# michalfratczak/habdec

Measured on AMD Instinct MI355X. Metric: IQ Msamples/s (batched 2.048 MS/s streams), higher is better.
Workload: dtype f32

## Files before the change

### habdec_amd/csrc/engine.cpp

```cpp
#include <hip/hip_runtime.h>
#include <rocfft/rocfft.h>

#include <algorithm>
#include <atomic>
#include <chrono>
#include <cmath>
#include <cstdio>
#include <cstdlib>
#include <cstring>
#include <memory>
#include <condition_variable>
#include <mutex>
#include <thread>
#include <string>
#include <vector>

#include "../../include/habdec_amd.h"
#include "dev_types.h"
#include "host/afc_tracker.hpp"
#include "host/decim_plan.hpp"
#include "host/fir_design.hpp"
#include "host/iq_file_batch.hpp"
#include "host/text_stage.hpp"
#include "host/tune_host.hpp"
#include "kernels/launch.h"

#define HDK(fn, ...) (e->fast ? hd::fast::fn(__VA_ARGS__) : hd::exact::fn(__VA_ARGS__))

namespace {

thread_local std::string g_err;
int fail(int code, const std::string& msg) { g_err = msg; return code; }

#define HD_HIP(call)                                                                                   \
    do {                                                                                               \
        hipError_t e_ = (call);                                                                        \
        if (e_ != hipSuccess) return fail(HD_ERR_DEVICE, std::string(#call) + ": " + hipGetErrorString(e_)); \
    } while (0)

template <typename T>
// ... 83 lines not shown
    int bins_sep = 8;
    bool decode_enabled = true;
    bool fast = false;
    bool one_stream = false;
    bool no_tail = false;
    uint32_t tail_max_n2 = 2048;
    int last_route = -1;
    struct PendingTail { bool valid = false; hd::TailArgs ta{}; int slot = 0; bool any_fft = false; int r2 = 0, t2 = 0; } pend;
    bool own_fft = false;
    bool tail_fft = true;
    DevBuf<float2> fft_tw;
    bool no_claim = false;
    uint32_t step_run = 0;
    bool no_cu_step = false;
    uint32_t ring_run = 0;
    uint32_t ring_short_pct = 25;
    static constexpr uint32_t kS1Loaders = 2;
#ifndef HD_S1_SLOTS_BATCH
#define HD_S1_SLOTS_BATCH 4
#endif
    static constexpr uint32_t kS1Slots = HD_S1_SLOTS_BATCH;
    PinBuf<unsigned int> ring_gave_up;
    std::string fail_cause;
    bool device_failed = false;
    uint64_t step_launches = 0;
    DevBuf<unsigned int> step_ctr;
    uint32_t pend_max_taps = 0;
    bool dec_wgs_forced = false;
#ifdef HD_TIMING_EXPERIMENT
    int cu_exp = 0;
// ... 160 lines not shown
        const float rel = (float)(500.0f / e->fsd);
        e->bins_sep = std::max(8, (int)std::round((double)rel * (double)hd::kFftBins));
    }

    int ndev = 0;
    if (hipGetDeviceCount(&ndev) != hipSuccess || ndev <= cfg->device || cfg->device < 0)
        return fail(HD_ERR_DEVICE, "no HIP device " + std::to_string(cfg->device) + " (this library has no CPU path)");
    HD_HIP(hipSetDevice(cfg->device));
    HD_HIP(hipStreamCreateWithFlags(&e->qa, hipStreamNonBlocking));
    e->one_stream = cfg->pipeline == 0;
    e->no_tail = getenv("HD_NO_TAIL") != nullptr;
    e->no_claim = getenv("HD_NO_CLAIM") != nullptr;
    if (const char* v = getenv("HD_STEP_RUN")) e->step_run = (uint32_t)atoi(v);
    e->no_cu_step = getenv("HD_NO_CU_STEP") != nullptr;
    if (const char* v = getenv("HD_RING_RUN")) e->ring_run = (uint32_t)atoi(v);
    if (const char* v = getenv("HD_RING_SHORT_PCT")) e->ring_short_pct = std::min<uint32_t>((uint32_t)atoi(v), 100u);
    if (const char* v = getenv("HD_TAIL_MAX_N2")) e->tail_max_n2 = (uint32_t)strtoul(v, nullptr, 0);
    {
        hipDeviceProp_t prop;
        HD_HIP(hipGetDeviceProperties(&prop, cfg->device));
        e->n_cus = (uint32_t)prop.multiProcessorCount;
        e->dec_wgs_per_cu = cfg->pipeline ? 6u : 8u;
        if (const char* v = getenv("HD_DEC_WGS_PER_CU")) { e->dec_wgs_per_cu = (uint32_t)atoi(v); e->dec_wgs_forced = true; }
#ifdef HD_TIMING_EXPERIMENT
        if (const char* v = getenv("HD_CU_EXP")) e->cu_exp = atoi(v);
#endif
    }
    for (hipEvent_t* ev : {&e->ev_copy[0], &e->ev_copy[1], &e->ev_staging_free[0], &e->ev_staging_free[1]}) HD_HIP(hipEventCreateWithFlags(ev, hipEventDisableTiming));
    if (e->one_stream) e->qb = e->qc = e->qa;
    else {
// ... 627 lines not shown
{
    t.dec1 = b.d1; t.dec1_stride = e->n1_cap; t.hist2_in = e->hist2[b.hin].p; t.hist2_out = e->hist2[b.hout].p; t.taps2 = e->stage_taps[1].p;
    t.fbuf = b.fcur; t.fbuf_next = b.fnext; t.fbuf_stride = e->fbuf_stride; t.fir_hist_cap = e->fir_hist_cap;
    t.lp_taps = e->lp_taps.p; t.taps_stride = e->taps_cap; t.demod = e->demod.p; t.demod_stride = e->demod.n / e->S;
    t.filtered = e->cfg.keep_filtered ? e->filtered.p : nullptr; t.carry_in = e->carry[b.cin].p; t.carry_out = e->carry[b.cout].p;
    t.tune = p.any_tune ? sl.h_tune.dev : nullptr; t.tune_tab = e->tune_tab.p;
    t.call = r.dcall; t.fft_in = r.feed; t.head_buf = e->fir_head.p; t.fbuf_prev = b.fprev; t.head_cap = e->head_cap;
    t.n_streams = e->S;
    t.ring = e->tail.p; t.ring_cap = e->tail_cap; t.sym = e->d_symstate.p; t.flipmask = e->flipmask.p; t.wsum = e->weight.p;
    t.sp = e->d_sym.p; t.slots = sl.h_slots.dev; t.slot_words = e->slot_words; t.seq = sl.seq;
    t.flips_dbg = e->flips_cap ? e->flips_dbg.p : nullptr; t.flips_cap = e->flips_cap;
    const bool in_tail = e->tail_fft && e->cfg.enable_spectrum && r.feed;
    t.fft_tw = in_tail ? e->fft_tw.p : nullptr; t.spec = e->spec.p; t.power = e->power.p; t.stats = sl.h_stats.dev; t.rate = e->fsd; t.bins_sep = e->bins_sep;
}

hd::StepClaim make_claim(const hd_engine* e, const CallPlan& p, uint32_t lin_wgs ,
                         uint32_t run_len_cu )
{
    hd::StepClaim claim{};
    const int R1 = (int)p.R1, T1 = (int)p.T1;
    const uint64_t S = e->S;
    const uint32_t ntiles = run_len_cu ? HDK(ring_tiles, R1, T1, p.max_in) : (p.max_n1 + 63) / 64, n_xcd = e->n_cus / 32u, run_len = run_len_cu ? run_len_cu : e->step_run >= 2 ? e->step_run : 4u;
    const uint64_t runs = S * ntiles / run_len;
    const bool shape_ok = run_len_cu ? (HDK(stage1_cu_supported, R1, T1) && p.max_in % 2048u == 0) : ((R1 == 32 || R1 == 64) && p.max_n1 % 64 == 0);
    if (!e->no_claim && (p.nst == 2 || (run_len_cu && p.nst == 1)) && shape_ok && p.min_in == p.max_in && p.max_in && !p.any_zero1 && n_xcd && e->n_cus % 32u == 0 && n_xcd <= 16 &&
        ntiles && (ntiles % run_len == 0 || (run_len_cu && R1 >= 32 && (S * ntiles) % run_len == 0)) && runs % n_xcd == 0 && S * ntiles < (1ull << 32) && (uint64_t)ntiles * S >= 4ull * lin_wgs) {
        claim.ctr = e->step_ctr.p + (size_t)(e->step_launches & 1u) * 16 * 32;
        claim.ctr_next = e->step_ctr.p + (size_t)((e->step_launches & 1u) ^ 1u) * 16 * 32;
        claim.n_xcd = n_xcd; claim.runs_per_xcd = (uint32_t)(runs / n_xcd); claim.run_len = run_len;
        if (run_len_cu && R1 >= 32 && e->ring_short_pct) {
            const uint32_t tpx = claim.runs_per_xcd * run_len, whole = (uint32_t)((uint64_t)tpx * (100u - e->ring_short_pct) / 100u) / run_len;
            claim.tiles_per_xcd = tpx; claim.short_from = whole; claim.runs_per_xcd = whole + (tpx - whole * run_len);
        }
    }
    return claim;
}

uint32_t pick_ring_run(const hd_engine* e, uint32_t R1, uint32_t ntiles)
{
    const uint64_t S = e->S;
    const uint32_t n_xcd = e->n_cus / 32u ? e->n_cus / 32u : 1u, want = R1 >= 32 ? 4u : 8u;
    auto ok = [&](uint32_t r) { return r >= 2u && r <= ntiles && (R1 >= 32 ? (S * ntiles) % r == 0 : ntiles % r == 0) && (S * ntiles / r) % n_xcd == 0; };
    if (e->ring_run >= 2 && ok(e->ring_run)) return e->ring_run;
    for (uint32_t d = 0; d <= 8u; ++d) {
        if (ok(want + d)) return want + d;
        if (d && d < want && ok(want - d)) return want - d;
    }
// ... 57 lines not shown
        hd::TailArgs tacu{};
        if (HDK(tail_layout, tacu, 64, R2, T2, p.max_taps, e->max_R, e->min_R, e->tail_cap, p.max_pend, cu_tail)) r.ta_step = tacu;
    }
    fill_tail(e, sl, p, r, b, r.ta_step);
    hd_engine::PendingTail prev = e->pend;
    hd_engine::CallSlot* ps = prev.valid ? &e->slot[prev.slot] : nullptr;
    bool ev_on_dispatch = false;
    const int cu_exp = e->cu_exp;
    const bool want_cu = cu_tail && ((cu_exp & 1) || (r.ta_step.lds_bytes <= cu_tail && (!prev.valid || prev.ta.lds_bytes <= cu_tail)));
    const hd::StepClaim claim = make_claim(e, p, 0, want_cu ? ring_run : 0u);
    bool launched = false;
    e->last_timing.step_variant = 0;
    if (want_cu && claim.ctr) {
        const uint32_t tb = std::max(r.ta_step.lds_bytes, prev.valid ? prev.ta.lds_bytes : 0u);
        hd::StepClaim cl = claim;
        if (cu_exp & 2) { cl.runs_per_xcd = 0; cl.tiles_per_xcd = 0; cl.short_from = 0xFFFFFFFFu; }
        ev_on_dispatch = !ps || prev.ta.fft_tw || !prev.any_fft;
        if (sl.timed && !ev_on_dispatch) HD_HIP(hipEventRecord(sl.t1, qa));
        launched = HDK(launch_step_cu, qa, R1, T1, prev.valid ? prev.r2 : R2, prev.valid ? prev.t2 : T2, S, e->n_cus, iq, stride,
                                      e->hist1[b.hin].p, e->hist1[b.hout].p, e->stage_taps[0].p, b.d1, e->n1_cap, sl.h_call.dev, sl.d_call.p, prev.ta,
                                      (prev.valid && !(cu_exp & 1)) ? S : 0u, p.max_in, cl, tb,
                                      ev_on_dispatch && sl.timed ? sl.t1 : nullptr, !ev_on_dispatch ? nullptr : sl.timed ? sl.t2 : ps ? ps->ev_done : nullptr);
        if (!launched && ev_on_dispatch) { ev_on_dispatch = false; if (sl.timed) HD_HIP(hipEventRecord(sl.t1, qa)); }
        e->last_timing.step_variant = launched ? 1u : 0u;
    }
    else if (sl.timed) HD_HIP(hipEventRecord(sl.t1, qa));
    if (launched) ++e->step_launches;
    else {
        const hd::StepClaim fb = (want_cu && claim.ctr) ? hd::StepClaim{} : claim;
        const uint32_t wgs = (fb.ctr ? 8u : 32u) * e->n_cus;
        if (prev.valid && prev.ta.lds_bytes > HDK(step_lds_bytes, R1, T1)) {
// ... 509 lines not shown
```

### habdec_amd/csrc/kernels/decimate.hip

```cpp
#include <hip/hip_runtime.h>
#include <hip/hip_ext.h>
#include <type_traits>
#include <cstdlib>

#include "launch.h"
#include "tune.h"
#include "tail_body.h"
#include "stage1_ring.h"

#define HD_DEC_MAXW 4

namespace hd {
namespace HD_ARITH_NS {

#ifdef HD_STAMP_DEC
#ifndef HD_STAMP_DEC_D
#define HD_STAMP_DEC_D 32
#endif
__device__ unsigned long long g_dec_stamps[4096 * 8];
extern "C" void HD_DBG_NAME(hd_debug_dec_stamps)(unsigned long long* host, size_t n) { (void)hipMemcpyFromSymbol(host, HIP_SYMBOL(g_dec_stamps), n * 8); }
#define DSTAMP_DECL unsigned long long ds_t = __builtin_amdgcn_s_memtime(), ds_acc[4] = {0, 0, 0, 0}; const unsigned long long ds_r0 = __builtin_amdgcn_s_memrealtime(); unsigned long long ds_r1 = 0
#define DSTAMP(i) do { if (D == HD_STAMP_DEC_D) { const unsigned long long t_ = __builtin_amdgcn_s_memtime(); ds_acc[i] += t_ - ds_t; ds_t = t_; } } while (0)
#define DSTAMP_ARRIVED() do { if (D == HD_STAMP_DEC_D) { asm volatile("s_waitcnt vmcnt(0)" ::: "memory"); DSTAMP(0); if (!ds_r1) ds_r1 = __builtin_amdgcn_s_memrealtime(); } } while (0)
#define DSTAMP_WRITE() do { if (D == HD_STAMP_DEC_D && threadIdx.x == 0) { const uint32_t w_ = by * gdx + bx; if (w_ < 4096) { \
// ... 620 lines not shown
                           out_stride, call, n_streams, ntiles, call_copy, ta, n_tail, uniform_n, claim);                             \
        return true;                                                                                                                  \
    }
    HD_STEP_CASE(32, 212, 2, 69) HD_STEP_CASE(32, 174, 4, 139) HD_STEP_CASE(64, 348, 4, 139)
#undef HD_STEP_CASE
    return false;
}

uint32_t ring_tiles(int ratio, int ntaps, uint32_t n)
{
    if (ratio != 32 && ratio != 64) return n / 2048u;
    const uint32_t adv = 64u - (uint32_t)((ntaps - 1 + ratio - 1) / ratio), rows = n / (uint32_t)ratio;
    return rows >= 64u ? (rows + adv - 1u) / adv : 0u;
}

static bool ring_limits_ok(uint32_t ntiles, const StepClaim& claim, bool workers = false )
{
    const uint64_t total = claim.tiles_per_xcd ? (uint64_t)claim.tiles_per_xcd * claim.n_xcd : (uint64_t)claim.runs_per_xcd * claim.n_xcd * claim.run_len;
    if (workers) return ntiles && claim.run_len >= 2u && total % ntiles == 0 && total < (1ull << 32) &&
                        (!claim.tiles_per_xcd || (uint64_t)claim.tiles_per_xcd == (uint64_t)(claim.short_from < claim.runs_per_xcd ? claim.short_from : claim.runs_per_xcd) * claim.run_len +
                                                                                    (claim.runs_per_xcd - (claim.short_from < claim.runs_per_xcd ? claim.short_from : claim.runs_per_xcd)));
    return ntiles && ntiles <= 4096u && claim.run_len && ntiles % claim.run_len == 0 && total < (1ull << 24) && total / ntiles <= (1ull << 20);
}

uint32_t step_cu_tail_lds(int ratio, int ntaps)
{
    if (ratio != 32 || (ntaps != 212 && ntaps != 174)) return 0;
    return ((163840u - (uint32_t)kRingCtlBytes - 4u * (uint32_t)kWorkSlotBytes) / 4u) & ~15u;
}

bool launch_step_cu(hipStream_t st, int ratio, int ntaps, int ratio2, int ntaps2, uint32_t n_streams, uint32_t n_cus, const float2* in, size_t in_stride,
                    const float2* hist_in, float2* hist_out, const float* taps, float2* out, size_t out_stride, const StreamCall* call,
                    StreamCall* call_copy, const TailArgs& ta, uint32_t n_tail, uint32_t uniform_n, const StepClaim& claim, uint32_t tail_bytes,
                    hipEvent_t ev_start, hipEvent_t ev_stop)
{
    if (ratio != 32 || !claim.ctr || !uniform_n || uniform_n % 2048u) return false;
    const uint32_t ntiles = ring_tiles(ratio, ntaps, uniform_n);
    if (!ring_limits_ok(ntiles, claim, true)) return false;
    if (tail_bytes < (uint32_t)kWorkSlotBytes) tail_bytes = (uint32_t)kWorkSlotBytes;
    tail_bytes = (tail_bytes + 15u) & ~15u;
    RingArgs ra{in, in_stride, hist_in, hist_out, taps, out, out_stride, uniform_n, ntiles, claim, nullptr, nullptr, 0u, nullptr};
#define HD_CU_CASE(T, D2, T2)                                                                                                         \
    if (ntaps == T && ratio2 == D2 && ntaps2 == T2) {                                                                                 \
        const uint32_t lds = (uint32_t)kRingCtlBytes + (n_tail ? 4u * (uint32_t)kWorkSlotBytes + 4u * tail_bytes : 8u * (uint32_t)kWorkSlotBytes); \
        if (lds > 163840u) return false;                                                                                              \
        static bool attr_set[64] = {};                              \
        int dev_ = 0;                                                                                                                 \
        if (hipGetDevice(&dev_) != hipSuccess || dev_ < 0 || dev_ >= 64) return false;                                                \
        if (!attr_set[dev_]) {                                                                                                        \
            if (hipFuncSetAttribute(reinterpret_cast<const void*>(k_step_cu<T, D2, T2>), hipFuncAttributeMaxDynamicSharedMemorySize, 163840) != hipSuccess) return false; \
            attr_set[dev_] = true;                                                                                                    \
        }                                                                                                                             \
        const dim3 grid_(n_cus > (n_streams + 3u) / 4u ? n_cus : (n_streams + 3u) / 4u);                                             \
// ... 18 lines not shown
}

bool launch_stage1_cu(hipStream_t st, int ratio, int ntaps, uint32_t n_cus, const float2* in, size_t in_stride, const float2* hist_in, float2* hist_out,
                      const float* taps, float2* out, size_t out_stride, uint32_t uniform_n, const StepClaim& claim, unsigned int* gave_up, uint32_t n_loaders, uint32_t n_waves,
                      uint32_t n_slots, const StreamCall* final_call, uint32_t fir_hist_cap, float2* fft_in)
{
    if (n_loaders != 1u) n_loaders = 2u;
    if (ratio <= 4) {
        n_loaders = 1u;
        n_waves = 16u;
    }
    if (n_slots < 2u * n_loaders || n_slots > 8u) n_slots = 8u;
    if (n_waves < 8u || n_waves > 16u) n_waves = 8u;
    if (!claim.ctr || !uniform_n || uniform_n % 2048u) return false;
    const uint32_t ntiles = ring_tiles(ratio, ntaps, uniform_n);
    if (!ring_limits_ok(ntiles, claim, ratio >= 32)) return false;
    if ((ratio <= 4) != (final_call != nullptr)) return false;
    RingArgs ra{in, in_stride, hist_in, hist_out, taps, out, out_stride, uniform_n, ntiles, claim, gave_up, final_call, fir_hist_cap, fft_in};
#define HD_S1_CASE(D, T)                                                                                                              \
    if (ratio == D && ntaps == T) {                                                                                                   \
        static_assert(D >= 32 || (uint32_t)ring_bytes<T, kRingNSLAlone>() <= 163840u, "eight tile slots must fit a CU's LDS");       \
        const uint32_t workers = D == 32 ? 8u : n_slots <= 4u ? 3u : 4u;             \
        const uint32_t lds = D >= 32 ? workers * (uint32_t)work_slot_bytes<(D >= 32 ? D : 32)>() : n_slots * (uint32_t)ring_slot_bytes<T>() + (uint32_t)kRingCtlBytes; \
        static bool attr_set[64] = {};                                                                                                \
        int dev_ = 0;                                                                                                                 \
        if (hipGetDevice(&dev_) != hipSuccess || dev_ < 0 || dev_ >= 64) return false;                                                \
        if (!attr_set[dev_]) {                                                                                                        \
            if (hipFuncSetAttribute(reinterpret_cast<const void*>(k_stage1_cu<T, D>), hipFuncAttributeMaxDynamicSharedMemorySize, 163840) != hipSuccess) return false; \
            attr_set[dev_] = true;                                                                                                    \
        }                                                                                                                             \
        hipLaunchKernelGGL((k_stage1_cu<T, D>), dim3(n_cus), dim3(64u * (D == 4 ? n_waves : D >= 32 ? workers : 8u)), lds, st, ra, n_loaders, n_slots);   \
// ... 33 lines not shown
```

### habdec_amd/csrc/kernels/launch.h

```cpp
#pragma once
#include <hip/hip_runtime.h>
#include <stddef.h>
#include <stdint.h>

#include "../dev_types.h"

namespace hd {

struct DemodCarry {
    float re, im;
    uint32_t primed;
    uint32_t _pad;
};

struct StepClaim {
    unsigned int* ctr = nullptr;
    unsigned int* ctr_next = nullptr;
    uint32_t n_xcd = 0, runs_per_xcd = 0, run_len = 0;
    uint32_t short_from = 0xFFFFFFFFu, tiles_per_xcd = 0;
};

struct TailArgs {
    const float2* dec1; size_t dec1_stride;
    const float2* hist2_in; float2* hist2_out; const float* taps2;
    float2* fbuf; float2* fbuf_next; size_t fbuf_stride; uint32_t fir_hist_cap;
    const float* lp_taps; uint32_t taps_stride;
    float* demod; size_t demod_stride; float2* filtered;
    const DemodCarry* carry_in; DemodCarry* carry_out;
    const StreamCall* call; float2* fft_in;
    float2* head_buf ; const float2* fbuf_prev ; uint32_t head_cap, n_streams;
    float* ring; uint32_t ring_cap; SymState* sym; unsigned long long* flipmask; float* wsum; const SymbolParams* sp;
    uint32_t* slots; uint32_t slot_words; uint32_t* flips_dbg; uint32_t flips_cap;
    uint32_t seq;
    const float2* fft_tw; float2* spec; float* power; SpectrumStatsDev* stats; double rate; int bins_sep;
// ... 24 lines not shown
```

### habdec_amd/csrc/kernels/stage1_ring.h

```cpp
#pragma once
#include <hip/hip_runtime.h>

#include "arith.h"
#include "launch.h"

namespace hd {
namespace HD_ARITH_NS {

typedef float r_f32x2 __attribute__((ext_vector_type(2)));
typedef float r_f32x4 __attribute__((ext_vector_type(4)));

constexpr int kRingRowBytes = 272;
constexpr int kRingNSLAlone = 4;
constexpr int kWorkSlotBytes = 64 * kRingRowBytes;
constexpr int kRingCtlBytes = 384;
constexpr uint32_t kRingSpinLimit = 1u << 22;
template <int T> constexpr int ring_halo_rows() { return (T - 1 + 31) / 32; }
template <int T> constexpr int ring_slot_bytes() { return (64 + ring_halo_rows<T>()) * kRingRowBytes; }
template <int T, int NSL = kRingNSLAlone> constexpr int ring_bytes() { return 2 * NSL * ring_slot_bytes<T>() + kRingCtlBytes; }
template <int T> constexpr int ring_adv() { return 64 - ring_halo_rows<T>(); }

__host__ __device__ constexpr uint32_t ring_sys_tiles(uint32_t n, uint32_t adv) { return (n / 32u + adv - 1u) / adv; }

#ifdef HD_STAMP_RING
// ... 73 lines not shown
}

__device__ __forceinline__ void glds16(const void* base, uint32_t off, uint32_t lds_dst)
{
    unsigned keep;
    asm volatile("s_mov_b32 %0, m0\n\ts_mov_b32 m0, %3\n\ts_nop 0\n\tglobal_load_lds_dwordx4 %1, %2\n\ts_mov_b32 m0, %0"
                 : "=&s"(keep) : "v"(off), "s"(base), "s"(lds_dst) : "memory");
}
__device__ __forceinline__ void glds4(const void* base, uint32_t off, uint32_t lds_dst)
{
    unsigned keep;
    asm volatile("s_mov_b32 %0, m0\n\ts_mov_b32 m0, %3\n\ts_nop 0\n\tglobal_load_lds_dword %1, %2\n\ts_mov_b32 m0, %0"
                 : "=&s"(keep) : "v"(off), "s"(base), "s"(lds_dst) : "memory");
}

template <bool HEAD_KEPT = false >
__device__ __forceinline__ void glds16_x17(const void* base, const uint32_t (&off)[17], uint32_t lds_dst)
{
    unsigned keep, scc_keep;
#define HD_GLDS_BODY_POLICY " nt"
#define HD_G1(n) "global_load_lds_dwordx4 %" #n ", %19" HD_GLDS_BODY_POLICY "\n\ts_add_u32 m0, m0, 0x400\n\ts_nop 0\n\t"
#define HD_G1D(n) "global_load_lds_dwordx4 %" #n ", %19\n\ts_add_u32 m0, m0, 0x400\n\ts_nop 0\n\t"
#define HD_G17_OPS : "=&s"(keep), "=&s"(scc_keep)                                                                                                                   \
                   : "v"(off[0]), "v"(off[1]), "v"(off[2]), "v"(off[3]), "v"(off[4]), "v"(off[5]), "v"(off[6]), "v"(off[7]), "v"(off[8]), "v"(off[9]),              \
                     "v"(off[10]), "v"(off[11]), "v"(off[12]), "v"(off[13]), "v"(off[14]), "v"(off[15]), "v"(off[16]), "s"(base), "s"(lds_dst)                      \
                   : "memory"
    if constexpr (HEAD_KEPT)
        asm volatile("s_cselect_b32 %1, 1, 0\n\ts_mov_b32 %0, m0\n\ts_mov_b32 m0, %20\n\ts_nop 0\n\t"
                     HD_G1D(2) HD_G1D(3) HD_G1(4) HD_G1(5) HD_G1(6) HD_G1(7) HD_G1(8) HD_G1(9) HD_G1(10) HD_G1(11) HD_G1(12) HD_G1(13) HD_G1(14) HD_G1(15) HD_G1(16) HD_G1D(17)
                     "global_load_lds_dwordx4 %18, %19\n\ts_mov_b32 m0, %0\n\ts_cmp_lg_u32 %1, 0" HD_G17_OPS);
    else
        asm volatile("s_cselect_b32 %1, 1, 0\n\ts_mov_b32 %0, m0\n\ts_mov_b32 m0, %20\n\ts_nop 0\n\t"
                     HD_G1(2) HD_G1(3) HD_G1(4) HD_G1(5) HD_G1(6) HD_G1(7) HD_G1(8) HD_G1(9) HD_G1(10) HD_G1(11) HD_G1(12) HD_G1(13) HD_G1(14) HD_G1(15) HD_G1(16) HD_G1D(17)
                     "global_load_lds_dwordx4 %18, %19\n\ts_mov_b32 m0, %0\n\ts_cmp_lg_u32 %1, 0" HD_G17_OPS);
#undef HD_G17_OPS
#undef HD_G1D
#undef HD_G1
}
template <int HR>
__device__ __forceinline__ void glds4_rows(const void* base, const uint32_t (&off)[HR], uint32_t lds_dst)
{
#pragma unroll
    for (int r = 0; r < HR; ++r) glds4(base, off[r], lds_dst + (uint32_t)r * kRingRowBytes);
}

__device__ __forceinline__ const void* uniform_ptr(const void* p)
{
    const uint64_t b = reinterpret_cast<uint64_t>(p);
    return reinterpret_cast<const void*>(((uint64_t)(uint32_t)__builtin_amdgcn_readfirstlane((int)(uint32_t)(b >> 32)) << 32) |
// ... 488 lines not shown
    const ctaps_t taps = (ctaps_t)(uintptr_t)a.taps - JS;
    const uint32_t dst = (uint32_t)__builtin_amdgcn_readfirstlane((int)lds_addr_of(slot));
    const unsigned char* p = slot + lane * (uint32_t)ROWB;
    const uint32_t rows = a.n / (uint32_t)D;
    RSTAMP_DECL;
    uint32_t n_done = 0; (void)n_done;

    uint32_t boff[CPR], hist_off[HR * HQ];
#pragma unroll
    for (int i = 0; i < CPR; ++i) { const uint32_t P = 64u * i + lane, row = P / (uint32_t)CPR, col = P - row * (uint32_t)CPR; boff[i] = row * (uint32_t)(D * 8) + (col < (uint32_t)(CPR - 1) ? col : (uint32_t)(CPR - 2)) * 16u; }
#pragma unroll
    for (int r = 0; r < HR * HQ; ++r) {
        const int h = (r / HQ - HR) * D + (r % HQ) * 32 + (int)(lane >> 1) + (T - 1);
        hist_off[r] = (uint32_t)(h < 0 ? 0 : h) * 8u + (lane & 1u) * 4u;
    }
    auto issue = [&](const uint32_t s, const uint32_t tile, const bool run_start) {
        const unsigned char* in_s = reinterpret_cast<const unsigned char*>(a.in + (size_t)s * a.in_stride);
        if (tile == 0) {
            const unsigned char* hb = reinterpret_cast<const unsigned char*>(a.hist_in + (size_t)s * (T - 1));
#pragma unroll
            for (int r = 0; r < HR * HQ; ++r) glds4(hb, hist_off[r], dst + (uint32_t)((r / HQ) * ROWB + (r % HQ) * 256));
#pragma unroll
            for (int i = 0; i < NB0; ++i)
                if (64 * (i + 1) <= (int)ADV * CPR || lane < (uint32_t)((int)ADV * CPR - 64 * i)) glds16(in_s, boff[i], dst + (uint32_t)(HR * ROWB) + 1024u * i);
        } else {
            const uint32_t origin = tile * ADV < rows - ADV ? tile * ADV : rows - ADV;
            const unsigned char* src = in_s + (size_t)(origin - (uint32_t)HR) * (uint32_t)(D * 8);
            if constexpr (D == 32) { if (run_start) glds16_x17<true>(src, boff, dst); else glds16_x17<false>(src, boff, dst); }
            else { glds16_x11<11>(src, boff, dst); glds16_x11<11>(src, boff + 11, dst + 11u * 1024u); glds16_x11<7>(src, boff + 22, dst + 22u * 1024u); }
        }
    };

    const uint32_t xcd0 = __builtin_amdgcn_s_getreg((3 << 11) | (0 << 6) | 20) & 15u;
    const uint32_t xcd = xcd0 < a.claim.n_xcd ? xcd0 : a.claim.n_xcd - 1;
    unsigned int* my_ctr = a.claim.ctr + (size_t)xcd * 32;
    unsigned int* next_ctr = a.claim.ctr_next + (size_t)xcd * 32;
    const uint32_t runs = a.claim.runs_per_xcd, run_len = a.claim.run_len, short_from = a.claim.short_from < runs ? a.claim.short_from : runs;
    const uint32_t tpx = a.claim.tiles_per_xcd ? a.claim.tiles_per_xcd : runs * run_len;
    auto draw = [&]() -> unsigned int { unsigned int t = 0; if (lane == 0) t = __hip_atomic_fetch_add(my_ctr, 1u, __ATOMIC_RELAXED, __HIP_MEMORY_SCOPE_AGENT); return t; };
    uint32_t s = 0, tile = 0, left = 0, this_run = 0;
    auto take_run = [&](const unsigned int ticket) -> bool {
        const uint32_t t = (uint32_t)__builtin_amdgcn_readfirstlane((int)ticket);
        if (t == runs && lane == 0) (void)__hip_atomic_exchange(next_ctr, 0u, __ATOMIC_RELAXED, __HIP_MEMORY_SCOPE_AGENT);
        if (t >= runs) return false;
        const uint32_t g0 = xcd * tpx + (t < short_from ? t * run_len : short_from * run_len + (t - short_from));
        s = g0 / a.ntiles; tile = g0 - s * a.ntiles; left = this_run = t < short_from ? run_len : 1u;
        return true;
    };
    auto advance = [&]() { ++tile; --left; if (tile == a.ntiles) { tile = 0; ++s; } };

    asm volatile("s_waitcnt lgkmcnt(0)" ::: "memory");
    if (!take_run(draw())) { RSTAMP_WRITE(role, 0); return; }
    uint32_t cs = s, ct = tile;
    issue(cs, ct, true); advance();
    unsigned int ticket = 0;
    if (!left) ticket = draw();

    auto ldk = [&](r_f32x2 (&k)[8], auto cc) {
        constexpr int c = decltype(cc)::value;
#pragma unroll
        for (int j = 0; j < 16; j += 2) {
            k[j >> 1].x = (16 * c + j >= JS && 16 * c + j < NS) ? taps[16 * c + j] : 0.f;
            k[j >> 1].y = (16 * c + j + 1 >= JS && 16 * c + j + 1 < NS) ? taps[16 * c + j + 1] : 0.f;
        }
    };
    for (;;) {
        RSTAMP(2);
        asm volatile("s_waitcnt vmcnt(0)" ::: "memory");
        asm volatile("" : "+v"(ticket));
        RSTAMP(0);
        r_f32x2 kk[2][2][8];
        r_f32x4 x[NX];
#pragma unroll
        for (int q = 0; q < NX; ++q) x[q] = *reinterpret_cast<const r_f32x4*>(p + 16 * q);
        ldk(kk[0][0], std::integral_constant<int, 0>{}); ldk(kk[0][1], std::integral_constant<int, 1>{});
        __builtin_amdgcn_sched_barrier(0);
#pragma unroll
        for (int q = 0; q < NX; q += 8)
            asm volatile("" : "+v"(x[q]), "+v"(x[q + 1]), "+v"(x[q + 2]), "+v"(x[q + 3]), "+v"(x[q + 4]), "+v"(x[q + 5]), "+v"(x[q + 6]), "+v"(x[q + 7]) :: "memory");
        RSTAMP(3);
        bool more = true;
        if (!left) more = take_run(ticket);
        uint32_t ns = 0, nt = 0;
        if (more) {
            ns = s; nt = tile;
            issue(ns, nt, left == this_run); advance();
            if (!left) ticket = draw();
        }
        RSTAMP(4);

        const uint32_t origin = ct * ADV < rows - ADV ? ct * ADV : rows - ADV;
        r_f32x2 acc = {0.f, 0.f};
#ifdef HD_FAST_ARITH
        r_f32x2 acc_b = {0.f, 0.f};
#endif
        auto mac_chunk = [&](const r_f32x2 (&k)[8], auto cc) {
            constexpr int c = decltype(cc)::value, j0 = JS > 16 * c ? JS - 16 * c : 0, j1 = NS < 16 * c + 16 ? NS - 16 * c : 16;
            const r_f32x4 (&xh)[8] = reinterpret_cast<const r_f32x4 (&)[8]>(x[8 * (c % (D / 16))]);
#ifdef HD_FAST_ARITH
            if constexpr (j0 == 0 && j1 == 16) ring_fma16x2(acc, acc_b, xh, k);
            else {
#pragma unroll
                for (int j = j0; j < j1; ++j) {
                    const r_f32x2 smp = (j & 1) ? xh[j >> 1].zw : xh[j >> 1].xy;
                    const float kj = (j & 1) ? k[j >> 1].y : k[j >> 1].x;
                    if (j & 1) acc_b = __builtin_elementwise_fma(smp, (r_f32x2){kj, kj}, acc_b);
// ... 4 lines not shown
            if constexpr (j0 == 0 && j1 == 16) ring_mac16_asm(acc, xh, k);
            else {
#pragma unroll
                for (int j = j0; j < j1; ++j) {
                    const r_f32x2 smp = (j & 1) ? xh[j >> 1].zw : xh[j >> 1].xy;
                    acc = acc + smp * ((j & 1) ? k[j >> 1].y : k[j >> 1].x);
                }
            }
#endif
        };
        auto rot1 = [&](r_f32x2& v) {
            const float re = v.x, im = v.y;
            v.x = __builtin_bit_cast(float, __builtin_amdgcn_update_dpp(0, __builtin_bit_cast(int, re), 0x13C, 0xF, 0xF, false));
            v.y = __builtin_bit_cast(float, __builtin_amdgcn_update_dpp(0, __builtin_bit_cast(int, im), 0x13C, 0xF, 0xF, false));
        };
        auto rot = [&]() {
            rot1(acc);
#ifdef HD_FAST_ARITH
            rot1(acc_b);
#endif
        };
        auto arrived = [&](const r_f32x2 (&k)[2][8]) {
            asm volatile("" :: "s"(k[0][0]), "s"(k[0][1]), "s"(k[0][2]), "s"(k[0][3]), "s"(k[0][4]), "s"(k[0][5]), "s"(k[0][6]), "s"(k[0][7]),
                               "s"(k[1][0]), "s"(k[1][1]), "s"(k[1][2]), "s"(k[1][3]), "s"(k[1][4]), "s"(k[1][5]), "s"(k[1][6]), "s"(k[1][7]));
        };
        ring_for_each_index([&](auto ui) {
            constexpr int u = decltype(ui)::value;
            arrived(kk[u & 1]);
            if constexpr (u + 1 < NU) {
                ldk(kk[(u + 1) & 1][0], std::integral_constant<int, 2 * u + 2>{});
                ldk(kk[(u + 1) & 1][1], std::integral_constant<int, 2 * u + 3>{});
            }
            __builtin_amdgcn_sched_barrier(0);
            if constexpr (JS < 32 * u + 16 && 32 * u < NS) mac_chunk(kk[u & 1][0], std::integral_constant<int, 2 * u>{});
            if constexpr (32 * u + 16 < NS && JS < 32 * u + 32) mac_chunk(kk[u & 1][1], std::integral_constant<int, 2 * u + 1>{});
            if constexpr ((u + 1) % UPS == 0 && u + 1 < NU) rot();
        }, std::make_integer_sequence<int, NU>{});
#ifdef HD_FAST_ARITH
        acc = acc + acc_b;
#endif
#ifdef HD_STAMP_RING
        asm volatile("" : "+v"(acc));
        ++n_done;
#endif
        RSTAMP(1);
        if (lane >= (uint32_t)HR) a.out[(size_t)cs * a.out_stride + origin + lane - (uint32_t)HR] = make_float2(acc.x, acc.y);
        if (ct + 1 == a.ntiles) {
            const float2* in_s = a.in + (size_t)cs * a.in_stride + (a.n - (uint32_t)(T - 1));
            float2* hout = a.hist_out + (size_t)cs * (T - 1);
            constexpr int NH = (T - 1 + 63) / 64;
            float2 h[NH];
#pragma unroll
            for (int k = 0; k < NH; ++k) h[k] = in_s[lane + 64u * k < (uint32_t)(T - 1) ? lane + 64u * k : 0u];
#pragma unroll
            for (int k = 0; k < NH; ++k) if (lane + 64u * k < (uint32_t)(T - 1)) hout[lane + 64u * k] = h[k];
        }
        if (!more) break;
        cs = ns; ct = nt;
    }
    RSTAMP(2);
    RSTAMP_WRITE(role, n_done);
}
// ... 4 lines not shown
```

Measured before the change: 479,200.

## Add chained ring runs and per-stream long/short ticket plan for stage-1 workers

```diff
diff --git a/habdec_amd/csrc/engine.cpp b/habdec_amd/csrc/engine.cpp
--- a/habdec_amd/csrc/engine.cpp
+++ b/habdec_amd/csrc/engine.cpp
@@ -24,6 +24,7 @@
 #include "host/text_stage.hpp"
 #include "host/tune_host.hpp"
 #include "kernels/launch.h"
+#include "kernels/ring_geom.h"
 
 #define HDK(fn, ...) (e->fast ? hd::fast::fn(__VA_ARGS__) : hd::exact::fn(__VA_ARGS__))
 
@@ -137,6 +138,7 @@
     uint32_t step_run = 0;
     bool no_cu_step = false;
     uint32_t ring_run = 0;
+    bool ring_chain = false;
     uint32_t ring_short_pct = 25;
     static constexpr uint32_t kS1Loaders = 2;
 #ifndef HD_S1_SLOTS_BATCH
@@ -327,6 +329,7 @@
     if (const char* v = getenv("HD_STEP_RUN")) e->step_run = (uint32_t)atoi(v);
     e->no_cu_step = getenv("HD_NO_CU_STEP") != nullptr;
     if (const char* v = getenv("HD_RING_RUN")) e->ring_run = (uint32_t)atoi(v);
+    if (const char* v = getenv("HD_RING_CHAIN")) e->ring_chain = atoi(v) != 0;
     if (const char* v = getenv("HD_RING_SHORT_PCT")) e->ring_short_pct = std::min<uint32_t>((uint32_t)atoi(v), 100u);
     if (const char* v = getenv("HD_TAIL_MAX_N2")) e->tail_max_n2 = (uint32_t)strtoul(v, nullptr, 0);
     {
@@ -984,6 +987,8 @@
     t.fft_tw = in_tail ? e->fft_tw.p : nullptr; t.spec = e->spec.p; t.power = e->power.p; t.stats = sl.h_stats.dev; t.rate = e->fsd; t.bins_sep = e->bins_sep;
 }
 
+constexpr uint32_t kRingRunWorkers = 4;
+
 hd::StepClaim make_claim(const hd_engine* e, const CallPlan& p, uint32_t lin_wgs ,
                          uint32_t run_len_cu )
 {
@@ -998,9 +1003,12 @@
         claim.ctr = e->step_ctr.p + (size_t)(e->step_launches & 1u) * 16 * 32;
         claim.ctr_next = e->step_ctr.p + (size_t)((e->step_launches & 1u) ^ 1u) * 16 * 32;
         claim.n_xcd = n_xcd; claim.runs_per_xcd = (uint32_t)(runs / n_xcd); claim.run_len = run_len;
-        if (run_len_cu && R1 >= 32 && e->ring_short_pct) {
-            const uint32_t tpx = claim.runs_per_xcd * run_len, whole = (uint32_t)((uint64_t)tpx * (100u - e->ring_short_pct) / 100u) / run_len;
-            claim.tiles_per_xcd = tpx; claim.short_from = whole; claim.runs_per_xcd = whole + (tpx - whole * run_len);
+        if (run_len_cu && R1 >= 32) {
+            const uint32_t len = e->ring_run >= 2u ? e->ring_run : kRingRunWorkers;
+            const hd::RingPlan plan = hd::ring_plan(p.max_in / (uint32_t)R1, (uint32_t)((T1 - 1 + R1 - 1) / R1), len, e->ring_chain);
+            const hd::RingTickets tk = hd::ring_tickets(plan, (uint32_t)S, e->ring_short_pct);
+            claim.run_len = len; claim.chain = e->ring_chain ? 1u : 0u; claim.streams = (uint32_t)S; claim.long_streams = tk.long_streams; claim.n_long = tk.n_long; claim.n_short = tk.n_short;
+            claim.runs_per_xcd = 0;
         }
     }
     return claim;
@@ -1088,7 +1096,7 @@
     if (want_cu && claim.ctr) {
         const uint32_t tb = std::max(r.ta_step.lds_bytes, prev.valid ? prev.ta.lds_bytes : 0u);
         hd::StepClaim cl = claim;
-        if (cu_exp & 2) { cl.runs_per_xcd = 0; cl.tiles_per_xcd = 0; cl.short_from = 0xFFFFFFFFu; }
+        if (cu_exp & 2) { cl.streams = cl.long_streams = cl.n_long = cl.n_short = 0; }
         ev_on_dispatch = !ps || prev.ta.fft_tw || !prev.any_fft;
         if (sl.timed && !ev_on_dispatch) HD_HIP(hipEventRecord(sl.t1, qa));
         launched = HDK(launch_step_cu, qa, R1, T1, prev.valid ? prev.r2 : R2, prev.valid ? prev.t2 : T2, S, e->n_cus, iq, stride,
diff --git a/habdec_amd/csrc/kernels/decimate.hip b/habdec_amd/csrc/kernels/decimate.hip
--- a/habdec_amd/csrc/kernels/decimate.hip
+++ b/habdec_amd/csrc/kernels/decimate.hip
@@ -658,13 +658,18 @@
     return rows >= 64u ? (rows + adv - 1u) / adv : 0u;
 }
 
-static bool ring_limits_ok(uint32_t ntiles, const StepClaim& claim, bool workers = false )
-{
-    const uint64_t total = claim.tiles_per_xcd ? (uint64_t)claim.tiles_per_xcd * claim.n_xcd : (uint64_t)claim.runs_per_xcd * claim.n_xcd * claim.run_len;
-    if (workers) return ntiles && claim.run_len >= 2u && total % ntiles == 0 && total < (1ull << 32) &&
-                        (!claim.tiles_per_xcd || (uint64_t)claim.tiles_per_xcd == (uint64_t)(claim.short_from < claim.runs_per_xcd ? claim.short_from : claim.runs_per_xcd) * claim.run_len +
-                                                                                    (claim.runs_per_xcd - (claim.short_from < claim.runs_per_xcd ? claim.short_from : claim.runs_per_xcd)));
+static bool ring_limits_ok(uint32_t ntiles, const StepClaim& claim)
+{
+    const uint64_t total = (uint64_t)claim.runs_per_xcd * claim.n_xcd * claim.run_len;
     return ntiles && ntiles <= 4096u && claim.run_len && ntiles % claim.run_len == 0 && total < (1ull << 24) && total / ntiles <= (1ull << 20);
+}
+static bool worker_claim_ok(int ratio, int ntaps, uint32_t n, const StepClaim& claim)
+{
+    const uint32_t rows = n / (uint32_t)ratio, hr = (uint32_t)((ntaps - 1 + ratio - 1) / ratio);
+    if (rows < 64u || !claim.n_xcd || claim.n_xcd > 16u || claim.run_len < 2u || claim.long_streams > claim.streams) return false;
+    const RingPlan plan = ring_plan(rows, hr, claim.run_len, claim.chain != 0u);
+    return plan.fresh_tiles && (uint64_t)claim.streams * plan.fresh_tiles < (1ull << 32) &&
+           (uint64_t)claim.n_long == (uint64_t)claim.long_streams * plan.runs && (uint64_t)claim.n_short == (uint64_t)(claim.streams - claim.long_streams) * plan.fresh_tiles;
 }
 
 uint32_t step_cu_tail_lds(int ratio, int ntaps)
@@ -680,7 +685,7 @@
 {
     if (ratio != 32 || !claim.ctr || !uniform_n || uniform_n % 2048u) return false;
     const uint32_t ntiles = ring_tiles(ratio, ntaps, uniform_n);
-    if (!ring_limits_ok(ntiles, claim, true)) return false;
+    if (!worker_claim_ok(ratio, ntaps, uniform_n, claim)) return false;
     if (tail_bytes < (uint32_t)kWorkSlotBytes) tail_bytes = (uint32_t)kWorkSlotBytes;
     tail_bytes = (tail_bytes + 15u) & ~15u;
     RingArgs ra{in, in_stride, hist_in, hist_out, taps, out, out_stride, uniform_n, ntiles, claim, nullptr, nullptr, 0u, nullptr};
@@ -729,7 +734,7 @@
     if (n_waves < 8u || n_waves > 16u) n_waves = 8u;
     if (!claim.ctr || !uniform_n || uniform_n % 2048u) return false;
     const uint32_t ntiles = ring_tiles(ratio, ntaps, uniform_n);
-    if (!ring_limits_ok(ntiles, claim, ratio >= 32)) return false;
+    if (ratio >= 32 ? !worker_claim_ok(ratio, ntaps, uniform_n, claim) : !ring_limits_ok(ntiles, claim)) return false;
     if ((ratio <= 4) != (final_call != nullptr)) return false;
     RingArgs ra{in, in_stride, hist_in, hist_out, taps, out, out_stride, uniform_n, ntiles, claim, gave_up, final_call, fir_hist_cap, fft_in};
 #define HD_S1_CASE(D, T)                                                                                                              \
diff --git a/habdec_amd/csrc/kernels/launch.h b/habdec_amd/csrc/kernels/launch.h
--- a/habdec_amd/csrc/kernels/launch.h
+++ b/habdec_amd/csrc/kernels/launch.h
@@ -17,7 +17,7 @@
     unsigned int* ctr = nullptr;
     unsigned int* ctr_next = nullptr;
     uint32_t n_xcd = 0, runs_per_xcd = 0, run_len = 0;
-    uint32_t short_from = 0xFFFFFFFFu, tiles_per_xcd = 0;
+    uint32_t chain = 0, streams = 0, long_streams = 0, n_long = 0, n_short = 0;
 };
 
 struct TailArgs {
diff --git a/habdec_amd/csrc/kernels/ring_geom.h b/habdec_amd/csrc/kernels/ring_geom.h
--- /dev/null
+++ b/habdec_amd/csrc/kernels/ring_geom.h
@@ -0,0 +1,123 @@
+#pragma once
+#include <stdint.h>
+
+#if defined(__HIPCC__)
+#define HD_GEOM_FN __host__ __device__ inline
+#else
+#define HD_GEOM_FN inline
+#endif
+
+namespace hd {
+
+struct RingPlan {
+    uint32_t rows, hr, adv, run_len;
+    uint32_t chained;
+    uint32_t runs;
+    uint32_t tiles;
+    uint32_t fresh_tiles;
+};
+struct RingRun {
+    uint32_t o0;
+    uint32_t n_grid;
+    uint32_t n_tail;
+    uint32_t step;
+};
+struct RingTile {
+    uint32_t origin;
+    uint32_t chained;
+};
+struct RingShare {
+    uint32_t lo_long, n_long, lo_short, n_short;
+};
+
+HD_GEOM_FN uint32_t ring_umin(uint32_t a, uint32_t b) { return a < b ? a : b; }
+
+HD_GEOM_FN RingRun ring_run(const RingPlan& p, uint32_t j)
+{
+    RingRun r;
+    if (!p.chained) {
+        const uint32_t t0 = j * p.run_len;
+        r.o0 = ring_umin(t0 * p.adv, p.rows - p.adv); r.n_grid = ring_umin(p.run_len, p.fresh_tiles - t0); r.n_tail = 0; r.step = p.adv;
+        return r;
+    }
+    const uint32_t w = p.adv + 64u * (p.run_len - 1u);
+    r.o0 = j * w; r.step = 64u; r.n_tail = 0;
+    const uint32_t rem = p.rows - r.o0;
+    if (rem < p.adv) { r.n_grid = 0; r.n_tail = 1; return r; }
+    r.n_grid = ring_umin(p.run_len, 1u + (rem - p.adv) / 64u);
+    if (r.n_grid < p.run_len) {
+        const uint32_t over = rem - (p.adv + 64u * (r.n_grid - 1u));
+        r.n_tail = over == 0 ? 0u : over <= p.adv ? 1u : 2u;
+    }
+    return r;
+}
+
+HD_GEOM_FN RingRun ring_single(const RingPlan& p, uint32_t t)
+{
+    RingRun r;
+    r.o0 = ring_umin(t * p.adv, p.rows - p.adv); r.n_grid = 1; r.n_tail = 0; r.step = p.adv;
+    return r;
+}
+
+HD_GEOM_FN RingTile ring_tile(const RingPlan& p, const RingRun& r, uint32_t k)
+{
+    RingTile t;
+    if (k < r.n_grid) { t.origin = ring_umin(r.o0 + k * r.step, p.rows - p.adv); t.chained = (r.step == 64u && k > 0) ? 1u : 0u; }
+    else { t.origin = k + 1u == r.n_grid + r.n_tail ? p.rows - p.adv : r.o0 + p.adv + 64u * (r.n_grid - 1u); t.chained = 0; }
+    return t;
+}
+
+HD_GEOM_FN RingPlan ring_plan(uint32_t rows, uint32_t hr, uint32_t run_len, bool chain)
+{
+    RingPlan p;
+    p.rows = rows; p.hr = hr; p.adv = 64u - hr; p.run_len = run_len ? run_len : 1u; p.chained = 0;
+    p.fresh_tiles = rows >= 64u ? (rows + p.adv - 1u) / p.adv : 0u;
+    p.runs = (p.fresh_tiles + p.run_len - 1u) / p.run_len; p.tiles = p.fresh_tiles;
+    if (chain && p.run_len >= 2u && p.fresh_tiles) {
+        const uint32_t w = p.adv + 64u * (p.run_len - 1u), runs = (rows + w - 1u) / w;
+        RingPlan c = p;
+        c.chained = 1; c.runs = runs;
+        const RingRun last = ring_run(c, runs - 1u);
+        c.tiles = (runs - 1u) * p.run_len + last.n_grid + last.n_tail;
+        if (c.tiles <= p.fresh_tiles) p = c;
+    }
+    return p;
+}
+
+HD_GEOM_FN RingShare ring_share(uint32_t total_long, uint32_t total_short, uint32_t n_xcd, uint32_t x)
+{
+    RingShare s;
+    s.lo_long = (uint32_t)((uint64_t)total_long * x / n_xcd); s.n_long = (uint32_t)((uint64_t)total_long * (x + 1u) / n_xcd) - s.lo_long;
+    s.lo_short = (uint32_t)((uint64_t)total_short * x / n_xcd); s.n_short = (uint32_t)((uint64_t)total_short * (x + 1u) / n_xcd) - s.lo_short;
+    return s;
+}
+
+HD_GEOM_FN uint32_t ring_long_streams(uint32_t n_streams, uint32_t short_pct)
+{
+    return (uint32_t)((uint64_t)n_streams * (100u - (short_pct < 100u ? short_pct : 100u)) / 100u);
+}
+
+struct RingTickets {
+    uint32_t long_streams, n_long, n_short;
+};
+HD_GEOM_FN RingTickets ring_tickets(const RingPlan& p, uint32_t streams, uint32_t short_pct)
+{
+    RingTickets t;
+    t.long_streams = ring_long_streams(streams, short_pct);
+    t.n_long = t.long_streams * p.runs; t.n_short = (streams - t.long_streams) * p.fresh_tiles;
+    return t;
+}
+
+HD_GEOM_FN RingRun ring_ticket(const RingPlan& p, const RingShare& share, uint32_t long_streams, uint32_t t, uint32_t& stream)
+{
+    if (t < share.n_long) {
+        const uint32_t g = share.lo_long + t;
+        stream = g / p.runs;
+        return ring_run(p, g - stream * p.runs);
+    }
+    const uint32_t g = share.lo_short + (t - share.n_long), q = g / p.fresh_tiles;
+    stream = long_streams + q;
+    return ring_single(p, g - q * p.fresh_tiles);
+}
+
+}
diff --git a/habdec_amd/csrc/kernels/stage1_ring.h b/habdec_amd/csrc/kernels/stage1_ring.h
--- a/habdec_amd/csrc/kernels/stage1_ring.h
+++ b/habdec_amd/csrc/kernels/stage1_ring.h
@@ -3,6 +3,7 @@
 
 #include "arith.h"
 #include "launch.h"
+#include "ring_geom.h"
 
 namespace hd {
 namespace HD_ARITH_NS {
@@ -111,7 +112,8 @@
                  : "=&s"(keep) : "v"(off), "s"(base), "s"(lds_dst) : "memory");
 }
 
-template <bool HEAD_KEPT = false >
+template <bool HEAD_KEPT = false ,
+          bool TAIL_KEPT = true >
 __device__ __forceinline__ void glds16_x17(const void* base, const uint32_t (&off)[17], uint32_t lds_dst)
 {
     unsigned keep, scc_keep;
@@ -122,14 +124,20 @@
                    : "v"(off[0]), "v"(off[1]), "v"(off[2]), "v"(off[3]), "v"(off[4]), "v"(off[5]), "v"(off[6]), "v"(off[7]), "v"(off[8]), "v"(off[9]),              \
                      "v"(off[10]), "v"(off[11]), "v"(off[12]), "v"(off[13]), "v"(off[14]), "v"(off[15]), "v"(off[16]), "s"(base), "s"(lds_dst)                      \
                    : "memory"
-    if constexpr (HEAD_KEPT)
-        asm volatile("s_cselect_b32 %1, 1, 0\n\ts_mov_b32 %0, m0\n\ts_mov_b32 m0, %20\n\ts_nop 0\n\t"
-                     HD_G1D(2) HD_G1D(3) HD_G1(4) HD_G1(5) HD_G1(6) HD_G1(7) HD_G1(8) HD_G1(9) HD_G1(10) HD_G1(11) HD_G1(12) HD_G1(13) HD_G1(14) HD_G1(15) HD_G1(16) HD_G1D(17)
-                     "global_load_lds_dwordx4 %18, %19\n\ts_mov_b32 m0, %0\n\ts_cmp_lg_u32 %1, 0" HD_G17_OPS);
+#define HD_G17_HEAD "s_cselect_b32 %1, 1, 0\n\ts_mov_b32 %0, m0\n\ts_mov_b32 m0, %20\n\ts_nop 0\n\t"
+#define HD_G17_MID HD_G1(4) HD_G1(5) HD_G1(6) HD_G1(7) HD_G1(8) HD_G1(9) HD_G1(10) HD_G1(11) HD_G1(12) HD_G1(13) HD_G1(14) HD_G1(15) HD_G1(16)
+#define HD_G17_END "\n\ts_mov_b32 m0, %0\n\ts_cmp_lg_u32 %1, 0"
+    if constexpr (HEAD_KEPT && TAIL_KEPT)
+        asm volatile(HD_G17_HEAD HD_G1D(2) HD_G1D(3) HD_G17_MID HD_G1D(17) "global_load_lds_dwordx4 %18, %19" HD_G17_END HD_G17_OPS);
+    else if constexpr (HEAD_KEPT)
+        asm volatile(HD_G17_HEAD HD_G1D(2) HD_G1D(3) HD_G17_MID HD_G1(17) "global_load_lds_dwordx4 %18, %19" HD_GLDS_BODY_POLICY HD_G17_END HD_G17_OPS);
+    else if constexpr (TAIL_KEPT)
+        asm volatile(HD_G17_HEAD HD_G1(2) HD_G1(3) HD_G17_MID HD_G1D(17) "global_load_lds_dwordx4 %18, %19" HD_G17_END HD_G17_OPS);
     else
-        asm volatile("s_cselect_b32 %1, 1, 0\n\ts_mov_b32 %0, m0\n\ts_mov_b32 m0, %20\n\ts_nop 0\n\t"
-                     HD_G1(2) HD_G1(3) HD_G1(4) HD_G1(5) HD_G1(6) HD_G1(7) HD_G1(8) HD_G1(9) HD_G1(10) HD_G1(11) HD_G1(12) HD_G1(13) HD_G1(14) HD_G1(15) HD_G1(16) HD_G1D(17)
-                     "global_load_lds_dwordx4 %18, %19\n\ts_mov_b32 m0, %0\n\ts_cmp_lg_u32 %1, 0" HD_G17_OPS);
+        asm volatile(HD_G17_HEAD HD_G1(2) HD_G1(3) HD_G17_MID HD_G1(17) "global_load_lds_dwordx4 %18, %19" HD_GLDS_BODY_POLICY HD_G17_END HD_G17_OPS);
+#undef HD_G17_HEAD
+#undef HD_G17_MID
+#undef HD_G17_END
 #undef HD_G17_OPS
 #undef HD_G1D
 #undef HD_G1
@@ -648,9 +656,9 @@
         const int h = (r / HQ - HR) * D + (r % HQ) * 32 + (int)(lane >> 1) + (T - 1);
         hist_off[r] = (uint32_t)(h < 0 ? 0 : h) * 8u + (lane & 1u) * 4u;
     }
-    auto issue = [&](const uint32_t s, const uint32_t tile, const bool run_start) {
+    auto issue = [&](const uint32_t s, const uint32_t origin, const bool head_kept, const bool tail_kept) {
         const unsigned char* in_s = reinterpret_cast<const unsigned char*>(a.in + (size_t)s * a.in_stride);
-        if (tile == 0) {
+        if (origin == 0) {
             const unsigned char* hb = reinterpret_cast<const unsigned char*>(a.hist_in + (size_t)s * (T - 1));
 #pragma unroll
             for (int r = 0; r < HR * HQ; ++r) glds4(hb, hist_off[r], dst + (uint32_t)((r / HQ) * ROWB + (r % HQ) * 256));
@@ -658,10 +666,14 @@
             for (int i = 0; i < NB0; ++i)
                 if (64 * (i + 1) <= (int)ADV * CPR || lane < (uint32_t)((int)ADV * CPR - 64 * i)) glds16(in_s, boff[i], dst + (uint32_t)(HR * ROWB) + 1024u * i);
         } else {
-            const uint32_t origin = tile * ADV < rows - ADV ? tile * ADV : rows - ADV;
             const unsigned char* src = in_s + (size_t)(origin - (uint32_t)HR) * (uint32_t)(D * 8);
-            if constexpr (D == 32) { if (run_start) glds16_x17<true>(src, boff, dst); else glds16_x17<false>(src, boff, dst); }
-            else { glds16_x11<11>(src, boff, dst); glds16_x11<11>(src, boff + 11, dst + 11u * 1024u); glds16_x11<7>(src, boff + 22, dst + 22u * 1024u); }
+            if constexpr (D == 32) {
+                if (head_kept) { if (tail_kept) glds16_x17<true, true>(src, boff, dst); else glds16_x17<true, false>(src, boff, dst); }
+                else { if (tail_kept) glds16_x17<false, true>(src, boff, dst); else glds16_x17<false, false>(src, boff, dst); }
+            } else {
+                glds16_x11<11>(src, boff, dst); glds16_x11<11>(src, boff + 11, dst + 11u * 1024u);
+                if (tail_kept) glds16_x11<7>(src, boff + 22, dst + 22u * 1024u); else glds16_x11<11>(src, boff + 22, dst + 22u * 1024u);
+            }
         }
     };
 
@@ -669,26 +681,37 @@
     const uint32_t xcd = xcd0 < a.claim.n_xcd ? xcd0 : a.claim.n_xcd - 1;
     unsigned int* my_ctr = a.claim.ctr + (size_t)xcd * 32;
     unsigned int* next_ctr = a.claim.ctr_next + (size_t)xcd * 32;
-    const uint32_t runs = a.claim.runs_per_xcd, run_len = a.claim.run_len, short_from = a.claim.short_from < runs ? a.claim.short_from : runs;
-    const uint32_t tpx = a.claim.tiles_per_xcd ? a.claim.tiles_per_xcd : runs * run_len;
+    const RingPlan plan = ring_plan(rows, (uint32_t)HR, a.claim.run_len, a.claim.chain != 0u);
+    const RingShare share = ring_share(a.claim.n_long, a.claim.n_short, a.claim.n_xcd, xcd);
+    const uint32_t runs = share.n_long + share.n_short;
     auto draw = [&]() -> unsigned int { unsigned int t = 0; if (lane == 0) t = __hip_atomic_fetch_add(my_ctr, 1u, __ATOMIC_RELAXED, __HIP_MEMORY_SCOPE_AGENT); return t; };
-    uint32_t s = 0, tile = 0, left = 0, this_run = 0;
+    uint32_t s = 0, k = 0, left = 0;
+    RingRun run = {0u, 0u, 0u, 64u};
     auto take_run = [&](const unsigned int ticket) -> bool {
         const uint32_t t = (uint32_t)__builtin_amdgcn_readfirstlane((int)ticket);
         if (t == runs && lane == 0) (void)__hip_atomic_exchange(next_ctr, 0u, __ATOMIC_RELAXED, __HIP_MEMORY_SCOPE_AGENT);
         if (t >= runs) return false;
-        const uint32_t g0 = xcd * tpx + (t < short_from ? t * run_len : short_from * run_len + (t - short_from));
-        s = g0 / a.ntiles; tile = g0 - s * a.ntiles; left = this_run = t < short_from ? run_len : 1u;
+        run = ring_ticket(plan, share, a.claim.long_streams, t, s);
+        k = 0; left = run.n_grid + run.n_tail;
         return true;
     };
-    auto advance = [&]() { ++tile; --left; if (tile == a.ntiles) { tile = 0; ++s; } };
+    auto issue_next = [&]() -> RingTile {
+        const RingTile t = ring_tile(plan, run, k);
+        issue(s, t.origin, k == 0, !(run.step == 64u && k + 1u < run.n_grid));
+        ++k; --left;
+        return t;
+    };
 
     asm volatile("s_waitcnt lgkmcnt(0)" ::: "memory");
     if (!take_run(draw())) { RSTAMP_WRITE(role, 0); return; }
-    uint32_t cs = s, ct = tile;
-    issue(cs, ct, true); advance();
+    uint32_t cs = s;
+    RingTile ct = issue_next();
     unsigned int ticket = 0;
     if (!left) ticket = draw();
+    r_f32x2 carry = {0.f, 0.f};
+#ifdef HD_FAST_ARITH
+    r_f32x2 carry_b = {0.f, 0.f};
+#endif
 
     auto ldk = [&](r_f32x2 (&k)[8], auto cc) {
         constexpr int c = decltype(cc)::value;
@@ -715,15 +738,16 @@
         RSTAMP(3);
         bool more = true;
         if (!left) more = take_run(ticket);
-        uint32_t ns = 0, nt = 0;
+        uint32_t ns = 0;
+        RingTile nt = {0u, 0u};
         if (more) {
-            ns = s; nt = tile;
-            issue(ns, nt, left == this_run); advance();
+            ns = s; nt = issue_next();
             if (!left) ticket = draw();
         }
         RSTAMP(4);
 
-        const uint32_t origin = ct * ADV < rows - ADV ? ct * ADV : rows - ADV;
+        const uint32_t origin = ct.origin;
+        const bool chained = ct.chained != 0u;
         r_f32x2 acc = {0.f, 0.f};
 #ifdef HD_FAST_ARITH
         r_f32x2 acc_b = {0.f, 0.f};
@@ -758,10 +782,25 @@
             v.x = __builtin_bit_cast(float, __builtin_amdgcn_update_dpp(0, __builtin_bit_cast(int, re), 0x13C, 0xF, 0xF, false));
             v.y = __builtin_bit_cast(float, __builtin_amdgcn_update_dpp(0, __builtin_bit_cast(int, im), 0x13C, 0xF, 0xF, false));
         };
-        auto rot = [&]() {
+        auto swap1 = [&](r_f32x2& v, r_f32x2& c, auto rr) {
+            constexpr int R = decltype(rr)::value;
+            const int vre = __builtin_bit_cast(int, (float)v.x), vim = __builtin_bit_cast(int, (float)v.y);
+            const int cre = __builtin_bit_cast(int, (float)c.x), cim = __builtin_bit_cast(int, (float)c.y);
+            const int nre = __builtin_amdgcn_readlane(vre, 0), nim = __builtin_amdgcn_readlane(vim, 0);
+            const int ore = __builtin_amdgcn_readlane(cre, R), oim = __builtin_amdgcn_readlane(cim, R);
+            c.x = lane == (uint32_t)R ? __builtin_bit_cast(float, nre) : c.x;
+            c.y = lane == (uint32_t)R ? __builtin_bit_cast(float, nim) : c.y;
+            if (chained) {
+                v.x = lane == 0u ? __builtin_bit_cast(float, ore) : v.x;
+                v.y = lane == 0u ? __builtin_bit_cast(float, oim) : v.y;
+            }
+        };
+        auto rot = [&](auto rr) {
             rot1(acc);
+            if (plan.chained) swap1(acc, carry, rr);
 #ifdef HD_FAST_ARITH
             rot1(acc_b);
+            if (plan.chained) swap1(acc_b, carry_b, rr);
 #endif
         };
         auto arrived = [&](const r_f32x2 (&k)[2][8]) {
@@ -778,7 +817,7 @@
             __builtin_amdgcn_sched_barrier(0);
             if constexpr (JS < 32 * u + 16 && 32 * u < NS) mac_chunk(kk[u & 1][0], std::integral_constant<int, 2 * u>{});
             if constexpr (32 * u + 16 < NS && JS < 32 * u + 32) mac_chunk(kk[u & 1][1], std::integral_constant<int, 2 * u + 1>{});
-            if constexpr ((u + 1) % UPS == 0 && u + 1 < NU) rot();
+            if constexpr ((u + 1) % UPS == 0 && u + 1 < NU) rot(std::integral_constant<int, (u + 1) / UPS>{});
         }, std::make_integer_sequence<int, NU>{});
 #ifdef HD_FAST_ARITH
         acc = acc + acc_b;
@@ -788,8 +827,8 @@
         ++n_done;
 #endif
         RSTAMP(1);
-        if (lane >= (uint32_t)HR) a.out[(size_t)cs * a.out_stride + origin + lane - (uint32_t)HR] = make_float2(acc.x, acc.y);
-        if (ct + 1 == a.ntiles) {
+        if (lane >= (uint32_t)HR || chained) a.out[(size_t)cs * a.out_stride + origin + lane - (uint32_t)HR] = make_float2(acc.x, acc.y);
+        if (origin == rows - ADV) {
             const float2* in_s = a.in + (size_t)cs * a.in_stride + (a.n - (uint32_t)(T - 1));
             float2* hout = a.hist_out + (size_t)cs * (T - 1);
             constexpr int NH = (T - 1 + 63) / 64;
```

Result: slower. 462,200 (-3.6%).
